# gorgonia/agogo

Hardware: AMD Instinct MI355X
Metric: mcts_sims_per_sec (higher is better)
Workload: dtype f32 (Winograd F(5x5,3x3): fp32 transforms; transform-domain products as fp16x2 = each fp32 operand scaled by a power of two and split into 2 fp16 pieces (22-23 significand bits, absolute error <= 2^-38 of the tensor range), 3 fp16 MFMAs per product, fp32 accumulate)

## Files before the change

agogo_amd/csrc/conv_wino_h2.hpp:

```cpp
#pragma once

template <int TM> struct WinoT;
template <> struct WinoT<4> {
  static constexpr int AL = 6, VSHIFT = 7;
  static constexpr float BT[6][6] = {{4, 0, -5, 0, 1, 0}, {0, -4, -4, 1, 1, 0}, {0, 4, -4, -1, 1, 0}, {0, -2, -1, 2, 1, 0}, {0, 2, -1, -2, 1, 0}, {0, 4, 0, -5, 0, 1}};
  static constexpr float AT[4][6] = {{1, 1, 1, 1, 1, 0}, {0, 1, -1, 2, -2, 0}, {0, 1, 1, 4, 4, 0}, {0, 1, -1, 8, -8, 1}};
  static constexpr double G[6][3] = {{1.0 / 4, 0, 0}, {-1.0 / 6, -1.0 / 6, -1.0 / 6}, {-1.0 / 6, 1.0 / 6, -1.0 / 6}, {1.0 / 24, 1.0 / 12, 1.0 / 6}, {1.0 / 24, -1.0 / 12, 1.0 / 6}, {0, 0, 1}};
};
template <> struct WinoT<5> {
  static constexpr int AL = 7, VSHIFT = 6;
  static constexpr float BT[7][7] = {{-0.5f, 0.25f, 2.5f, -1.25f, -2, 1, 0}, {0, 0.5f, 0.25f, -2.25f, -1, 1, 0}, {0, -0.5f, 0.75f, 1.75f, -3, 1, 0},
                                     {0, 1, 1.5f, -2, -1.5f, 1, 0},          {0, -1, 2.5f, 0, -2.5f, 1, 0},       {0, 0.25f, 0, -1.25f, 0, 1, 0},
                                     {0, -0.5f, 0.25f, 2.5f, -1.25f, -2, 1}};
  static constexpr float AT[5][7] = {{1, 1, 1, 1, 1, 1, 0}, {0, 1, -1, 0.5f, -0.5f, 2, 0}, {0, 1, 1, 0.25f, 0.25f, 4, 0}, {0, 1, -1, 0.125f, -0.125f, 8, 0},
                                     {0, 1, 1, 0.0625f, 0.0625f, 16, 1}};
  static constexpr double G[7][3] = {{-2, 0, 0}, {-2.0 / 3, -2.0 / 3, -2.0 / 3}, {-2.0 / 9, 2.0 / 9, -2.0 / 9}, {16.0 / 9, 8.0 / 9, 4.0 / 9}, {16.0 / 15, -8.0 / 15, 4.0 / 15},
                                     {2.0 / 45, 4.0 / 45, 8.0 / 45}, {0, 0, 1}};
};
template <int TM> __device__ __forceinline__ void wino_btv(const float* d, float* o);
template <int TM> __device__ __forceinline__ void wino_atv(const float* m, float* o);
template <> __device__ __forceinline__ void wino_btv<4>(const float* d, float* o) { wino_bt6(d, o); }
template <> __device__ __forceinline__ void wino_atv<4>(const float* m, float* o) { wino_at4(m, o); }
template <> __device__ __forceinline__ void wino_btv<5>(const float* d, float* o) {
  o[0] = -0.5f * d[0] + 0.25f * d[1] + 2.5f * d[2] - 1.25f * d[3] - 2.f * d[4] + d[5];
// ... 31 lines not shown
  const unsigned* amax_in;
  unsigned* amax_out;
  float* wave_max;
  float w_unscale;
  const float* t_in;
  const float* col_unscale;
  const float* t_next;
  int cform;
  const _Float16* U2c;
  const float* amax_true;
  const float* wm_prev;
  float* wm_out;
  unsigned* amax_next;
  float g1, g0;
  int gemm_variant;
  int temporal_stores;
  int live_r, live_c;
  int row_pad;
};
__device__ __forceinline__ size_t h2_row(const WinoH2Args& h, int pos, int t) {
  return (size_t)(t >> h.rsh) * h.rA + (size_t)pos * h.rB + (size_t)(t & h.rmask);
}

__device__ __forceinline__ void wino_h2_scales(unsigned amax_bits, int shift, float* s, float* inv) {
  int e = (int)((amax_bits >> 23) & 0xffu);
  if (amax_bits == 0u) { *s = 1.f; *inv = 1.f; return; }
  e = e < 30 ? 30 : (e > 230 ? 230 : e);
  *s = __uint_as_float((unsigned)(268 - shift - e) << 23);
  *inv = __uint_as_float((unsigned)(e - 14 + shift) << 23);
}
// ... 1072 lines not shown
```

agogo_amd/csrc/conv_wino_h2c.hpp:

```cpp
#pragma once

__device__ __forceinline__ unsigned h2c_img(int row, int slot) { return maps::h2c_img(row, slot); }

template <int NK, int PFA>
__global__ __launch_bounds__(256, 2) void wino_gemm_h2c_kernel(WinoH2Args h) {
  const WinoArgs& a = h.w;
  constexpr int SA = 128 * 128, SB = 256 * 128;
  __shared__ __attribute__((aligned(16))) unsigned char lds[SA + SB];

  const int n_nt = a.Ntot >> 8;
  const int per_pos = a.n_mtiles * n_nt;
  const int nblk = h.npos * per_pos;
  const int id = blockIdx.x;
  int q = nblk >> 3, rr = nblk & 7, xcd = id & 7, slot = id >> 3;
  int tile = (xcd < rr ? xcd * (q + 1) : rr * (q + 1) + (xcd - rr) * q) + slot;
  const int pos = tile / per_pos;
  const int rem = tile - pos * per_pos;
  const int m_tile = rem / n_nt, n_tile = rem - m_tile * n_nt;

  const int tid = threadIdx.x, lane = tid & 63, wid = tid >> 6;
  const int wm = wid >> 1, wn = wid & 1;
  const unsigned st_lds = h2c_img(tid >> 3, tid & 7);
  const char* abase = reinterpret_cast<const char*>(a.V) + ((size_t)m_tile * h.npos + pos) * (size_t)NK * SA + (size_t)tid * 16;
  const char* bbase = reinterpret_cast<const char*>(h.U2c) + (((size_t)pos * NK) * n_nt + n_tile) * (size_t)SB + (size_t)tid * 16;
// ... 521 lines not shown
template <> __device__ __forceinline__ void wino_atv_p<4>(const f2c* m, f2c* o) {
  const f2c s12 = m[1] + m[2], d12 = m[1] - m[2], s34 = m[3] + m[4], d34 = m[3] - m[4];
  o[0] = m[0] + s12 + s34;
  o[1] = d12 + 2.f * d34;
  o[2] = s12 + 4.f * s34;
  o[3] = d12 + 8.f * d34 + m[5];
}
template <> __device__ __forceinline__ void wino_atv_p<5>(const f2c* m, f2c* o) {
  const f2c s12 = m[1] + m[2], d12 = m[1] - m[2], s34 = m[3] + m[4], d34 = m[3] - m[4];
  o[0] = m[0] + s12 + s34 + m[5];
  o[1] = d12 + 0.5f * d34 + 2.f * m[5];
  o[2] = s12 + 0.25f * s34 + 4.f * m[5];
  o[3] = d12 + 0.125f * d34 + 8.f * m[5];
  o[4] = s12 + 0.0625f * s34 + 16.f * m[5] + m[6];
}
template <int TM> __device__ __forceinline__ void wino_at_acc_p(int nu, f2c* Y, f2c t);
template <> __device__ __forceinline__ void wino_at_acc_p<5>(int nu, f2c* Y, f2c t) {
  switch (nu) {
    case 0: Y[0] += t; break;
    case 1: Y[0] += t; Y[1] += t; Y[2] += t; Y[3] += t; Y[4] += t; break;
    case 2: Y[0] += t; Y[1] -= t; Y[2] += t; Y[3] -= t; Y[4] += t; break;
    case 3: Y[0] += t; Y[1] += 0.5f * t; Y[2] += 0.25f * t; Y[3] += 0.125f * t; Y[4] += 0.0625f * t; break;
    case 4: Y[0] += t; Y[1] -= 0.5f * t; Y[2] += 0.25f * t; Y[3] -= 0.125f * t; Y[4] += 0.0625f * t; break;
    case 5: Y[0] += t; Y[1] += 2.f * t; Y[2] += 4.f * t; Y[3] += 8.f * t; Y[4] += 16.f * t; break;
    default: Y[4] += t; break;
  }
}
template <> __device__ __forceinline__ void wino_at_acc_p<4>(int nu, f2c* Y, f2c t) {
  switch (nu) {
    case 0: Y[0] += t; break;
// ... 19 lines not shown
template <> __device__ __forceinline__ f2c wino_bt_row_p<4>(int i, const f2c* d) {
  switch (i) {
    case 0: return 4.f * d[0] - 5.f * d[2] + d[4];
    case 1: return -4.f * d[1] - 4.f * d[2] + d[3] + d[4];
    case 2: return 4.f * d[1] - 4.f * d[2] - d[3] + d[4];
    case 3: return -2.f * d[1] - d[2] + 2.f * d[3] + d[4];
    case 4: return 2.f * d[1] - d[2] - 2.f * d[3] + d[4];
    default: return 4.f * d[1] - 5.f * d[3] + d[5];
  }
}
template <int TM> __device__ __forceinline__ void wino_btv_p(const f2c* d, f2c* o) {
#pragma unroll
  for (int i = 0; i < TM + 2; i++) o[i] = wino_bt_row_p<TM>(i, d);
}

template <int TM, bool NT = true>
__global__ __launch_bounds__(256, 2) void wino_oip_h2c_kernel(WinoH2Args h) {
  constexpr int MAUX = 0, VAUX = NT ? 2 : 0;
  using WT = WinoT<TM>;
  constexpr int AL = WT::AL, NPRE = AL - 3;
  const WinoArgs& a = h.w;
  extern __shared__ __attribute__((aligned(16))) float ys[];
  const int tid = threadIdx.x, tl = tid >> 4, pr = tid & 15, lane = tid & 63;
  const int NS = a.C >> 5;
  const int PH = TM * a.nty + 2, PW = TM * a.ntx + 2;
  const int bpg = 16 / a.TPB;
  const int n_groups = (a.T + 15) >> 4, n_items = n_groups * NS;
  const int tt = tl % a.TPB, bl = tl / a.TPB;
  const int ty = tt / a.ntx, tx = tt - ty * a.ntx;
  for (int i = tid; i < bpg * PH * PW * 32; i += 256) ys[i] = 0.f;
  const __amdgpu_buffer_rsrc_t mr = h2_rsrc(a.Mb);
// ... 54 lines not shown
    for (int k = 0; k < TM; k++)
#pragma unroll
      for (int l = 0; l < TM; l++) { Y[k][l][0] = f2c{0.f, 0.f}; Y[k][l][1] = f2c{0.f, 0.f}; }
#pragma unroll
    for (int nu = 0; nu < AL; nu++) {
      f2c c0[AL], c1[AL], o0[TM], o1[TM];
#pragma unroll
      for (int xi = 0; xi < AL; xi++) {
        const float4 v = m[nu % NPRE][xi];
        c0[xi] = f2c{v.x, v.y}; c1[xi] = f2c{v.z, v.w};
      }
      if (nu + NPRE < AL) {
#pragma unroll
        for (int xi = 0; xi < AL; xi++) m[nu % NPRE][xi] = h2_ldf4<MAUX>(mr, m_voff(xi, nu + NPRE), m_soff(g, s, xi, nu + NPRE));
      }
      wino_atv_p<TM>(c0, o0);
      wino_atv_p<TM>(c1, o1);
#pragma unroll
      for (int k = 0; k < TM; k++) {
        f2c y0[TM], y1[TM];
#pragma unroll
        for (int l = 0; l < TM; l++) { y0[l] = Y[k][l][0]; y1[l] = Y[k][l][1]; }
        wino_at_acc_p<TM>(nu, y0, o0[k]);
        wino_at_acc_p<TM>(nu, y1, o1[k]);
#pragma unroll
        for (int l = 0; l < TM; l++) { Y[k][l][0] = y0[l]; Y[k][l][1] = y1[l]; }
      }
      __builtin_amdgcn_sched_barrier(0);
    }
    __builtin_amdgcn_sched_barrier(0);
    unsigned e_base = (unsigned)(32 * s + 2 * pr) * 16u + (unsigned)((TM * ty) * a.W + TM * tx) * e_pix;
    asm volatile("" : "+v"(e_base));
// ... 16 lines not shown
      if (k + 1 < TM) load_e((k + 1) & 1, k + 1);
#pragma unroll
      for (int l = 0; l < TM; l++) {
        const bool ok = live && ((okmask >> (k * TM + l)) & 1u);
        const float4 E0 = E[k & 1][l][0], E1 = E[k & 1][l][1];
        const f2c u0 = Y[k][l][0] * un0, u1 = Y[k][l][1] * un0;
        float va = u0.x * E0.x + E0.y, vb = u0.y * E0.z + E0.w;
        float vc = u1.x * E1.x + E1.y, vd = u1.y * E1.z + E1.w;
        va = va > 0.f ? va : 0.f; vb = vb > 0.f ? vb : 0.f; vc = vc > 0.f ? vc : 0.f; vd = vd > 0.f ? vd : 0.f;
        const float y0 = ok ? va + vb : 0.f, y1 = ok ? vc + vd : 0.f;
        *reinterpret_cast<float2*>(yw + ((k + 1) * PW + l + 1) * 32) = make_float2(y0, y1);
        mxv = fmaxf(mxv, fmaxf(y0, y1));
      }
      __builtin_amdgcn_sched_barrier(0);
    }
#pragma unroll
    for (int o = 8; o > 0; o >>= 1) mxv = fmaxf(mxv, __shfl_xor(mxv, o, 64));
    if (pr == 0 && live) h.wm_out[(size_t)t * NS + s] = mxv;
    float ax;
    if (h.amax_true) ax = __uint_as_float(reinterpret_cast<const unsigned*>(h.amax_true)[b]);
    else {
      const int wmpb = a.TPB * NS;
      const float* wp = h.wm_prev + (size_t)b * wmpb;
      ax = 0.f;
      for (int i = pr; i < wmpb; i += 16) ax = fmaxf(ax, wp[i]);
#pragma unroll
      for (int o = 8; o > 0; o >>= 1) ax = fmaxf(ax, __shfl_xor(ax, o, 64));
    }
    const float bound = h.g1 * ax + h.g0;
    const unsigned bbits = __float_as_uint(bound);
    if (s == 0 && tt == 0 && pr == 0 && live) h.amax_next[b] = bbits;
    float sb, inv_;
    wino_h2_scales(bbits, WT::VSHIFT, &sb, &inv_);
    const float sv = live ? sb : 0.f;
    __syncthreads();
    {
      const int nx = item + (int)gridDim.x < n_items ? item + (int)gridDim.x : item;
      const int g2 = __builtin_amdgcn_readfirstlane(nx / NS), s2 = __builtin_amdgcn_readfirstlane(nx - (nx / NS) * NS);
#pragma unroll
      for (int nu = 0; nu < NPRE; nu++)
#pragma unroll
        for (int xi = 0; xi < AL; xi++) m[nu][xi] = h2_ldf4<MAUX>(mr, m_voff(xi, nu), m_soff(g2, s2, xi, nu));
    }
    __builtin_amdgcn_sched_barrier(0);
    const unsigned v_base = (unsigned)((((g >> 3) * h.npos) * NS + s)) * 16384u;
    const unsigned v_g = (unsigned)(g & 7) * 2048u, v_g_r = (unsigned)(g & 7) * (gr_r * 128u), v_g_c = (unsigned)(g & 7) * (gr_c * 128u);
    const unsigned v_pos = (unsigned)NS * 16384u;
    const float* yr = ybase;
    asm volatile("" : "+v"(yr));
#pragma unroll
    for (int i0 = 0; i0 < AL; i0 += 3) {
      constexpr int NRMAX = 3;
      const int nr = AL - i0 < NRMAX ? AL - i0 : NRMAX;
      f2c tmr[NRMAX][AL];
#pragma unroll
      for (int j = 0; j < AL; j++) {
        f2c d[AL];
#pragma unroll
        for (int ii = 0; ii < AL; ii++) {
// ... 59 lines not shown
  h.tm = tm; h.npos = (tm + 2) * (tm + 2);
  a.nty = ceil_div(a.H, tm); a.ntx = ceil_div(a.W, tm); a.TPB = a.nty * a.ntx; a.T = a.B * a.TPB;
  h.rsh = 7; h.rmask = 127; h.rA = (unsigned)h.npos * 128u; h.rB = 128u;
  a.n_mtiles = ceil_div(a.T, 128); a.n_ntiles = ceil_div(a.Ntot, 128);
  h.in_swap = 1; h.cform = 1; h.wm_per_board = 0;
}
constexpr int WINO_H2_GEMM_DEFAULT = 1;
static inline int wino_h2c_gemm_variant(const WinoH2Args& h) { return h.gemm_variant > 0 ? h.gemm_variant : WINO_H2_GEMM_DEFAULT; }
static inline bool wino_h2c_dma_ok(const WinoH2Args& h) {
  return wino_h2_rows(h.npos, (size_t)h.w.T) * h.w.C * 4 < ((size_t)1 << 31) && (size_t)h.npos * h.w.C * h.w.Ntot * 4 < ((size_t)1 << 31);
}
static inline bool wino_h2c_fits31(const WinoH2Args& h) { return wino_h2_rows(h.npos, (size_t)h.w.T) * h.w.Ntot * 4 < ((size_t)1 << 31); }
static bool wino_h2c_oip_ready(agz_ctx* ctx) {
  if (!(ctx->func_attr_state & 2u)) {
    const bool ok = hipFuncSetAttribute(reinterpret_cast<const void*>(&wino_oip_h2c_kernel<5>), hipFuncAttributeMaxDynamicSharedMemorySize, 80 * 1024) == hipSuccess &&
                    hipFuncSetAttribute(reinterpret_cast<const void*>(&wino_oip_h2c_kernel<4>), hipFuncAttributeMaxDynamicSharedMemorySize, 80 * 1024) == hipSuccess;
    if (!ok) (void)hipGetLastError();
    ctx->func_attr_state |= 2u | (ok ? 1u : 0u);
  }
  return (ctx->func_attr_state & 1u) != 0;
}
static void wino_h2c_rows(agz_ctx* ctx, WinoH2Args& h, int oi_variant, bool keep_all) {
  wino_h2c_geometry(h);
  h.live_r = h.live_c = 0;
  const int gemm = wino_h2c_gemm_variant(h) & 15;
  const maps::WinoRows g = maps::wino_rows(h.w.H, h.w.W, h.tm);
  if (keep_all || gemm != 1 || oi_variant != 4 || !wino_h2c_dma_ok(h) || !wino_h2c_fits31(h) || !maps::rows_short_ok(g) || !wino_h2c_oip_ready(ctx)) return;
  h.live_r = g.dead_y ? maps::rows_slot_live(g, maps::ROWS_R) : 0;
  h.live_c = g.dead_x ? maps::rows_slot_live(g, maps::ROWS_C) : 0;
}
static void wino_h2c_in(agz_ctx* ctx, WinoH2Args& h, hipStream_t st) {
// ... 33 lines not shown
  }
  switch (h.w.C >> 5) {
    case 4: hipLaunchKernelGGL((wino_gemm_h2c_kernel<4, 2>), g, dim3(256), 0, st, h); break;
    case 8: hipLaunchKernelGGL((wino_gemm_h2c_kernel<8, 2>), g, dim3(256), 0, st, h); break;
    case 12: hipLaunchKernelGGL((wino_gemm_h2c_kernel<12, 2>), g, dim3(256), 0, st, h); break;
    default: hipLaunchKernelGGL((wino_gemm_h2c_kernel<16, 2>), g, dim3(256), 0, st, h); break;
  }
}
static void wino_h2c_oi(agz_ctx* ctx, WinoH2Args& h, bool last, hipStream_t st, int variant = 4) {
  wino_h2c_geometry(h);
  ProfScopeOn ps(ctx, AGZ_PROF_WINO_OUT, st == ctx->stream.raw());
  const WinoArgs& a = h.w;
  const dim3 g((unsigned)ceil_div(a.T, 16), (unsigned)(a.C >> 5));
  const size_t shm = last ? 0 : (size_t)(16 / a.TPB) * a.H * a.W * 32 * sizeof(float);
  const bool fits31 = wino_h2c_fits31(h);
  if (variant == 4 && !last && fits31 && wino_h2c_oip_ready(ctx)) {
    const size_t shp = (size_t)(16 / a.TPB) * (h.tm * a.nty + 2) * (h.tm * a.ntx + 2) * 32 * sizeof(float);
    const int items = ceil_div(a.T, 16) * (a.C >> 5);
    const dim3 gp((unsigned)std::min(items, 2 * ctx->num_cus));
    if (h.tm == 5 && h.temporal_stores) {
      (void)hipFuncSetAttribute(reinterpret_cast<const void*>(&wino_oip_h2c_kernel<5, false>), hipFuncAttributeMaxDynamicSharedMemorySize, 80 * 1024);
      hipLaunchKernelGGL((wino_oip_h2c_kernel<5, false>), gp, dim3(256), shp, st, h);
      return;
    }
    if (h.tm == 5) hipLaunchKernelGGL((wino_oip_h2c_kernel<5>), gp, dim3(256), shp, st, h);
    else hipLaunchKernelGGL((wino_oip_h2c_kernel<4>), gp, dim3(256), shp, st, h);
    return;
  }
  if (h.tm == 5) {
    if (last) hipLaunchKernelGGL((wino_oi_h2c_kernel<5, true>), g, dim3(256), shm, st, h);
    else hipLaunchKernelGGL((wino_oi_h2c_kernel<5, false>), g, dim3(256), shm, st, h);
  } else {
    if (last) hipLaunchKernelGGL((wino_oi_h2c_kernel<4, true>), g, dim3(256), shm, st, h);
    else hipLaunchKernelGGL((wino_oi_h2c_kernel<4, false>), g, dim3(256), shm, st, h);
// ... 3 lines not shown
```

agogo_amd/csrc/conv_x3.hpp:

```cpp
#pragma once

typedef short bf16x8_t __attribute__((ext_vector_type(8)));
typedef unsigned u32x4_t __attribute__((ext_vector_type(4)));

__device__ __forceinline__ void x3_split(float v, unsigned& h, unsigned& m, unsigned& l) {
  unsigned hu = __float_as_uint(v) & 0xffff0000u;
  float r = v - __uint_as_float(hu);
  unsigned mu = __float_as_uint(r) & 0xffff0000u;
  float r2 = r - __uint_as_float(mu);
  h = hu; m = mu; l = __float_as_uint(r2);
}
__device__ __forceinline__ unsigned x3_pack(unsigned e0, unsigned e1) { return __builtin_amdgcn_perm(e1, e0, 0x07060302u); }

__device__ __forceinline__ unsigned x3_lds_off(int row, int half) { return (unsigned)(row * 32 + ((half ^ ((row >> 3) & 1)) << 4)); }

__device__ __forceinline__ void x3_amax_flush(unsigned* amax, int b, float m, int lane) {
#pragma unroll
  for (int o = 16; o > 0; o >>= 1) m = fmaxf(m, __shfl_xor(m, o, 64));
  if ((lane & 31) == 0) atomicMax(&amax[b], __float_as_uint(m));
}
#define X3_EPILOGUE \
  int amx_b = -1; float amx_m = 0.f;    \
  _Pragma("unroll") \
  for (int i = 0; i < 2; i++) { \
// ... 30 lines not shown
              a.y[obase + c] = acc[i][j][r]; \
            } else { \
              float2 e = reinterpret_cast<const float2*>(a.ep)[(size_t)p * a.Cout_p + c]; \
              float v = acc[i][j][r] * e.x + e.y; \
              v = v > 0.f ? v : 0.f; \
              a.y[obase + c] = v; \
              amx_m = fmaxf(amx_m, v); \
            } \
          } \
        } \
      } \
    } \
  } \
  if (!DUAL && a.amax_out && amx_b >= 0) x3_amax_flush(a.amax_out, amx_b, amx_m, lane);

template <bool DUAL>
__global__ __launch_bounds__(256, 3) void conv3x3_x3_kernel(ConvArgs a, const unsigned short* __restrict__ w3) {
  constexpr int BM = 128, BNT = 128;
  constexpr int PIECE = 128 * 32;
  constexpr int STAGE = 6 * PIECE;
  __shared__ __attribute__((aligned(16))) unsigned char lds[2 * STAGE];

  const int nblk = a.n_mtiles * a.n_ntiles;
  const int id = blockIdx.x;
  int q = nblk >> 3, rr = nblk & 7, xcd = id & 7, slot = id >> 3;
  int tile = (xcd < rr ? xcd * (q + 1) : rr * (q + 1) + (xcd - rr) * q) + slot;
  const int m_tile = tile / a.n_ntiles, n_tile = tile - m_tile * a.n_ntiles;
  const int m0 = m_tile * BM, n0 = n_tile * BNT;

  const int tid = threadIdx.x, lane = tid & 63, wid = tid >> 6;
// ... 100 lines not shown
    X3_STORE_B(XB0, XB1, XB2, (BUF) ^ 1) X3_SB                                               \
    X3_QUAD(0, 1) X3_QUAD(0, 0) X3_SB                                                        \
    __syncthreads();                                                                         \
  }

  X3_GLOAD(ya0, ya1, yb0, yb1, yb2)
  X3_GLOAD(xa0, xa1, xb0, xb1, xb2)
  X3_STORE_A(ya0, ya1, 0)
  X3_STORE_B(yb0, yb1, yb2, 0)
  __syncthreads();
  for (int it = 0; it < NK; it += 2) {
    X3_ITER(0, xa0, xa1, xb0, xb1, xb2, ya0, ya1, yb0, yb1, yb2)
    if (it + 1 < NK) X3_ITER(1, ya0, ya1, yb0, yb1, yb2, xa0, xa1, xb0, xb1, xb2)
  }

  X3_EPILOGUE
}
```

agogo_amd/csrc/net.hip:

```cpp
#include "net.hpp"
#include "gemm_maps.hpp"

#include <cmath>
#include <cstdio>
#include <cstring>
#include <type_traits>

typedef float f32x16 __attribute__((ext_vector_type(16)));
typedef float f32x4 __attribute__((ext_vector_type(4)));

namespace agz {

struct ConvArgs {
  const float* x;
  const float* w;
  const void* ep;
  float* y;
  int M, HW, W, Wp, HpWp;
  int Cin_p, Cout_p, Ntot;
  int n_mtiles, n_ntiles;
  int raw;
  int splits;
  int per;
  float* ws;
  const unsigned* amax_in;
  float w_unscale;
  const unsigned* w_amax_dev;
  unsigned* amax_out;
};

__device__ __forceinline__ int swz_off(int row, int chunk) { return row * 32 + ((chunk ^ ((row >> 1) & 7)) << 2); }

template <int WM, int WN, int MT, bool DUAL>
__device__ __forceinline__ void conv_tile(const ConvArgs& a, float* lds, const int m0, const int n_tile, const int split) {
  constexpr int BM = WM * MT * 32;
  constexpr int BNT = WN * 64;
  static_assert(WM * WN == 4, "4 waves");
  constexpr int STAGE = (BM + BNT) * 32;
  const int n0 = n_tile * BNT;

  const int tid = threadIdx.x, lane = tid & 63, wid = tid >> 6;
  const int wm = wid / WN, wn = wid % WN;

// ... 1046 lines not shown
    wino_v_cap = t.v_elems * t.n_scr; wino_chunk_cap = 0;
  }
  const size_t need_amax = (size_t)(conf.SharedLayers + 1) * B + t.wm_board * B;
  if (need_amax > amax_cap) {
    AGZ_HIP_TRY(hipStreamSynchronize(ctx->stream));
    if (ctx->stream2) AGZ_HIP_TRY(hipStreamSynchronize(ctx->stream2));
    if (d_amax) hipFree(d_amax);
    d_amax = nullptr; amax_cap = 0;
    AGZ_HIP_TRY(hipMalloc(&d_amax, need_amax * sizeof(unsigned)));
    amax_cap = need_amax;
    if (amax_moved) *amax_moved = true;
  }
  return AGZ_OK;
}

void agz_net::wino_h2c_block(int l, int B, int b0, int ci, const H2Tower& t, hipStream_t st, float* cur, float* nxt) {
  const size_t wmb = (size_t)t.tpb * (Kp >> 5);
  const bool last = l + 1 == conf.SharedLayers;
  float* d_wave_max = reinterpret_cast<float*>(d_amax + (size_t)(conf.SharedLayers + 1) * B);
  WinoH2Args hh{};
  WinoArgs& wa = hh.w;
  wa.x = cur + (size_t)b0 * Hp * Wp * Kp; wa.y = nxt + (size_t)b0 * Hp * Wp * Kp;
  wa.V = d_wV + (size_t)ci * t.v_elems; wa.Mb = d_wM + (size_t)ci * t.m_elems; wa.ep = d_ep_h2[l];
  wa.B = std::min(t.chunk, B - b0); wa.H = H; wa.W = W; wa.Hp = Hp; wa.Wp = Wp; wa.C = Kp; wa.Cout_p = Kp; wa.Ntot = 2 * Kp;
  hh.U2c = d_u2c_dual[l]; hh.w_unscale = 1.f; hh.tm = wino_tm;
  hh.amax_in = d_amax + (size_t)l * B + b0;
  hh.amax_next = last ? nullptr : d_amax + (size_t)(l + 1) * B + b0;
  hh.amax_true = l == 0 ? reinterpret_cast<const float*>(d_amax + b0) : nullptr;
  hh.wm_prev = d_wave_max + ((size_t)((l + 1) & 1) * B + b0) * wmb;
  hh.wm_out = d_wave_max + ((size_t)(l & 1) * B + b0) * wmb;
  hh.g1 = wino_g1[l]; hh.g0 = wino_g0[l];
  {
    static const int gemm_env = [] {
      const char* e = getenv("AGZ_WINO_H2_GEMM");
      const int v = e ? atoi(e) : 0;
      if (v == 0 || (((v & 63) == 1 || (v & 63) == 2) && (v >> 6) <= 3)) return v;
      fprintf(stderr, "libagz: AGZ_WINO_H2_GEMM=%s ignored (want 1 or 2, optionally + 64 and / or + 128)\n", e);
      return 0;
    }();
    const int gv = wino_gemm > 0 ? wino_gemm : gemm_env;
    hh.gemm_variant = gv & 63; hh.temporal_stores = (gv >> 6) & 1;
    agz::wino_h2c_rows(ctx, hh, t.form_want == 1 ? 1 : 4, ((gv >> 7) & 1) != 0);
    wino_live_r = hh.live_r; wino_live_c = hh.live_c;
  }
  if (l == 0) agz::wino_h2c_in(ctx, hh, st);
  agz::wino_h2c_gemm(ctx, hh, st);
  agz::wino_h2c_oi(ctx, hh, last, st, t.form_want == 1 ? 1 : 4);
}

void agz_net::heads_spread_range(agz::HeadArgs h, bool nb4, int B, int b0, int nb, hipStream_t st) {
  h.x += (size_t)b0 * Hp * Wp * Kp;
  h.feat = d_hs + (size_t)b0 * 3 * HW; h.cols = d_hs + (size_t)B * 3 * HW + (size_t)b0 * (conf.ActionSpace + conf.FC);
  h.policy += (size_t)b0 * conf.ActionSpace; h.value += b0;
  hipLaunchKernelGGL(heads_feat_kernel, dim3(ceil_div(HW, 4), nb), dim3(256), 0, st, h);
  if (nb4)
    hipLaunchKernelGGL(heads_fc_nb_kernel<4>, dim3(ceil_div(conf.ActionSpace + conf.FC, 64), ceil_div(nb, 4)), dim3(1024), 0, st, h, nb);
  else
    hipLaunchKernelGGL(heads_fc_kernel, dim3(ceil_div(conf.ActionSpace + conf.FC, 64), nb), dim3(1024), 0, st, h);
  hipLaunchKernelGGL(heads_out_kernel, dim3(nb), dim3(256), 0, st, h);
}

// ... 24 lines not shown
  }
  return AGZ_OK;
}

int agz_net::forward_half(int B, int half, hipStream_t st, float* policy_dev, float* value_dev, hipEvent_t mid) {
  const int nb = B / 2, b0 = half * nb;
  const FwdPlan plan = fwd_plan(B);
  const H2Tower t = wino_h2_tower(B);
  ConvArgs a{};
  a.M = nb * HW; a.HW = HW; a.W = W; a.Wp = Wp; a.HpWp = Hp * Wp;
  a.x = d_act_in + (size_t)b0 * Hp * Wp * Fp; a.w = d_w_init; a.ep = d_ep_init_h2; a.y = d_actA + (size_t)b0 * Hp * Wp * Kp;
  a.Cin_p = Fp; a.Cout_p = Kp; a.Ntot = Kp;
  a.n_ntiles = ceil_div(a.Ntot, 128); a.n_mtiles = ceil_div(a.M, 128);
  a.splits = 1; a.per = 0; a.ws = nullptr; a.raw = 0;
  AGZ_HIP_TRY(hipMemsetAsync(d_amax + b0, 0, (size_t)nb * sizeof(unsigned), st));
  a.amax_out = d_amax + b0;
  hipLaunchKernelGGL((conv3x3_x3_kernel<false>), dim3(a.n_mtiles * a.n_ntiles), dim3(256), 0, st, a, d_w3_init);
  const int L = conf.SharedLayers;
  for (int l = 0; l < L; l++) {
    wino_h2c_block(l, B, b0, half, t, st, d_actA, d_actB);
    if (mid && l == L / 2) AGZ_HIP_TRY(hipEventRecord(mid, st));
  }
  HeadArgs h{};
  h.x = d_actB; h.conv = d_head_conv; h.bn = d_head_bn; h.Wp = d_Wp; h.bp = d_bp; h.W1 = d_W1; h.b1 = d_b1; h.W2 = d_W2;
  h.b2 = d_b2; h.policy = policy_dev; h.value = value_dev;
  h.H = H; h.W = W; h.HW = HW; h.Wp_ = Wp; h.HpWp = Hp * Wp; h.Kp = Kp; h.A = conf.ActionSpace; h.FC = conf.FC;
  heads_spread_range(h, plan.heads_nb, B, b0, nb, st);
  AGZ_HIP_TRY(hipGetLastError());
  return AGZ_OK;
}

// ... 33 lines not shown
    lat_wmax_cap = B;
  }
  int rc;
  bool amax0_done = false;
  if (lat_in) {
    agz::LatInArgs li{};
    li.x = d_act_in; li.w = d_w_init_t; li.ep = reinterpret_cast<const float2*>(d_ep_init); li.t = d_lat_tin[0]; li.y = d_actA; li.words = d_lat_wmax[1];
    li.B = B; li.H = H; li.W = W; li.Hp = Hp; li.Wp = Wp; li.Cout_p = Kp; li.groups_per_board = in_groups;
    ProfScope ps(ctx, AGZ_PROF_CONV_INIT);
    hipLaunchKernelGGL(agz::lat_input_kernel, dim3(Kp / 64, B * in_groups), dim3(256), 0, ctx->stream, li);
    rc = AGZ_OK;
  }
  else if (split_ok && compute_mode != AGZ_COMPUTE_F32_MFMA && d_w3_init && Kp % 128 == 0 &&
      (size_t)B * Hp * Wp * Fp * sizeof(float) < ((size_t)1 << 32)) {
    a.n_ntiles = ceil_div(a.Ntot, 128); a.n_mtiles = ceil_div(a.M, 128);
    a.splits = 1; a.per = 0; a.ws = nullptr; a.raw = 0;
    ProfScope ps(ctx, AGZ_PROF_CONV_INIT);
    if (wino_h2_ok && d_amax && amax_cap >= (size_t)B) {
      AGZ_HIP_TRY(hipMemsetAsync(d_amax, 0, (size_t)B * sizeof(unsigned), ctx->stream));
      a.amax_out = d_amax; amax0_done = true;
    }
    hipLaunchKernelGGL((conv3x3_x3_kernel<false>), dim3(a.n_mtiles * a.n_ntiles), dim3(256), 0, ctx->stream, a, d_w3_init);
    a.amax_out = nullptr;
    rc = AGZ_OK;
  }
  else if (cfg != 0) rc = launch_conv<4, 1, 1, false>(ctx, a, wsp, &ws_cap);
  else if (half_init) rc = launch_conv<2, 2, 1, false>(ctx, a, wsp, &ws_cap);
  else rc = launch_conv<2, 2, 2, false>(ctx, a, wsp, &ws_cap);
  if (rc != AGZ_OK) return rc;
  float* cur = d_actA;
  float* nxt = d_actB;
// ... 514 lines not shown
int agz_net_min_same_batch(agz_net* n, int k, int G, int* batch) {
  AGZ_REQUIRE(n && batch && k >= 1 && G >= k, AGZ_E_INVALID, "agz_net_min_same_batch: bad argument");
  AGZ_REQUIRE(n->committed, AGZ_E_STATE, "agz_net_min_same_batch: commit the net first");
  *batch = n->min_same_batch(k, G);
  return AGZ_OK;
}

int agz_net_wino_h2_last_rows(agz_net* n, int* live_r, int* live_c) {
  AGZ_REQUIRE(n && live_r && live_c, AGZ_E_INVALID, "agz_net_wino_h2_last_rows: null argument");
  *live_r = n->wino_live_r; *live_c = n->wino_live_c;
  return AGZ_OK;
}

int agz_net_set_wino_h2_gemm(agz_net* n, int variant) {
  AGZ_REQUIRE(n, AGZ_E_INVALID, "agz_net_set_wino_h2_gemm: null net");
  AGZ_REQUIRE(((variant & 63) <= 2 && (variant >> 6) <= 3) || ((variant & 15) == 2 && (variant >> 4) <= 3), AGZ_E_INVALID, "agz_net_set_wino_h2_gemm: variant %d (want 0, 1, 2, + 64, + 128, or 2 + 16 * mode)", variant);
  n->wino_gemm = variant;
  return AGZ_OK;
}

int agz_wino_stages(agz_ctx* ctx, const float* x, const float* w, int B, int H, int W, int C, int N, float* V, float* M) {
  AGZ_REQUIRE(ctx && x && w && V && M, AGZ_E_INVALID, "agz_wino_stages: NULL argument");
  AGZ_REQUIRE(B >= 1 && H >= 1 && W >= 1 && C >= 16 && C % 16 == 0 && N >= 1, AGZ_E_INVALID, "agz_wino_stages: bad shape");
  AGZ_HIP_TRY(hipSetDevice(ctx->device));
  const int Hp = H + 2, Wp = W + 2;
  std::vector<float> xp((size_t)B * Hp * Wp * C, 0.f);
  for (int b = 0; b < B; b++) for (int h = 0; h < H; h++)
    memcpy(&xp[(((size_t)b * Hp + h + 1) * Wp + 1) * C], &x[((size_t)b * H + h) * W * C], (size_t)W * C * sizeof(float));
  std::vector<unsigned short> u3;
  agz::wino_build_u3(u3, N, C, [&](int n, int ci, int tap) -> double { return (double)w[((size_t)n * C + ci) * 9 + tap]; });
  agz::WinoArgs a{};
// ... 128 lines not shown
```

agogo_amd/csrc/net.hpp:

```cpp
#pragma once
#include <string>
#include <vector>

#include "common.hpp"

namespace agz {
struct Param {
  std::string name;
  std::vector<float> v;
  std::vector<int> ref_shape;
  int kind;
};
struct BNStats { std::vector<float> mean, var; };
int conv3x3_raw(agz_ctx* ctx, const float* x, const float* w, float* y, int B, int H, int W, int Cin_p, int Cout_p);
int conv3x3_raw_x3(agz_ctx* ctx, const float* x, const unsigned short* w3, float* y, int B, int H, int W, int Cin_p, int Cout_p);
int split_w3(agz_ctx* ctx, const float* w, unsigned short* w3, int N, int Cin_p);
inline size_t w3_elems(int N, int Cin_p) { return (size_t)9 * 3 * N * Cin_p; }
struct WinoRawScratch {
  float* V = nullptr; float* M = nullptr; void* U2 = nullptr; unsigned* words = nullptr;
  size_t v_cap = 0, m_cap = 0, u_cap = 0; int b_cap = 0;
  void* w2 = nullptr; unsigned* h2_words = nullptr;
  size_t w2_cap = 0; int h2_b_cap = 0, h2_flip = 0;
};
int conv3x3_raw_h2(agz_ctx* ctx, const float* x, const float* w, float* y, int B, int H, int W, int Cin_p, int Cout_p, WinoRawScratch* sc,
// ... 28 lines not shown
  float* d_ep_init = nullptr;
  unsigned short* d_w3_init = nullptr;
  std::vector<float*> d_w_dual;
  std::vector<float*> d_ep_dual;
  std::vector<unsigned short*> d_w3_dual;
  std::vector<_Float16*> d_w2_dual;
  std::vector<float> w_unscale;
  std::vector<unsigned short*> d_u3_dual;
  std::vector<_Float16*> d_u2_dual;
  std::vector<float> u_unscale;
  std::vector<float*> d_u2_tin;
  std::vector<float*> d_u2_colun;
  std::vector<_Float16*> d_u2c_dual;
  std::vector<float> wino_g1, wino_g0;
  int wino_gemm = 0;
  int wino_live_r = 0, wino_live_c = 0;
  int wino_form = -1;
  void free_u2c() { for (auto& p : d_u2c_dual) if (p) hipFree(p); d_u2c_dual.clear(); wino_g1.clear(); wino_g0.clear(); }
  int build_wino_h2_weights();
  int wino_tm = 4;
  size_t wino_v_cap = 0;
  float* d_wV = nullptr;
  float* d_wM = nullptr;
  int wino_chunk_cap = 0;
  int build_wino_weights();
  unsigned* d_amax = nullptr;
  size_t amax_cap = 0;
  int compute_mode = AGZ_COMPUTE_F32_MFMA;
  bool compute_force = false;
  float* d_head_conv = nullptr;
// ... 47 lines not shown
```

Before: 44300.

## Route last Winograd layer through OIP kernel and add row-wise x3 epilogue

Adds a LAST template variant of the in-place output-transform kernel that skips the amax/scale computation for the next layer and writes the final tower output directly from shared memory. It also adds a row-wise epilogue for the initial x3 conv that uses permlane32 swaps and readlane-indexed per-row epilogue params, plus a new gemm-word bit (256) that selects the old paths. By default (bit clear) the last layer now uses the OIP path and the x3 kernel uses the new epilogue. The aim is to avoid a separate slower last-layer output kernel and unnecessary amax work, at the cost of extra kernel instantiations and a scalar-heavy epilogue.

Result: no change. 44470 (median of 6 runs) (+0.4%).

```diff
diff --git a/agogo_amd/csrc/conv_wino_h2.hpp b/agogo_amd/csrc/conv_wino_h2.hpp
--- a/agogo_amd/csrc/conv_wino_h2.hpp
+++ b/agogo_amd/csrc/conv_wino_h2.hpp
@@ -69,6 +69,7 @@
   unsigned* amax_next;
   float g1, g0;
   int gemm_variant;
+  int last_plain;
   int temporal_stores;
   int live_r, live_c;
   int row_pad;
diff --git a/agogo_amd/csrc/conv_wino_h2c.hpp b/agogo_amd/csrc/conv_wino_h2c.hpp
--- a/agogo_amd/csrc/conv_wino_h2c.hpp
+++ b/agogo_amd/csrc/conv_wino_h2c.hpp
@@ -559,6 +559,12 @@
   o[3] = d12 + 0.125f * d34 + 8.f * m[5];
   o[4] = s12 + 0.0625f * s34 + 16.f * m[5] + m[6];
 }
+__device__ __forceinline__ void wino_atv_p4_seq(const f2c* m, f2c* o) {
+  o[0] = m[0] + m[1] + m[2] + m[3] + m[4];
+  o[1] = m[1] - m[2] + 2.f * m[3] - 2.f * m[4];
+  o[2] = m[1] + m[2] + 4.f * m[3] + 4.f * m[4];
+  o[3] = m[1] - m[2] + 8.f * m[3] - 8.f * m[4] + m[5];
+}
 template <int TM> __device__ __forceinline__ void wino_at_acc_p(int nu, f2c* Y, f2c t);
 template <> __device__ __forceinline__ void wino_at_acc_p<5>(int nu, f2c* Y, f2c t) {
   switch (nu) {
@@ -608,7 +614,7 @@
   for (int i = 0; i < TM + 2; i++) o[i] = wino_bt_row_p<TM>(i, d);
 }
 
-template <int TM, bool NT = true>
+template <int TM, bool NT = true, bool LAST = false>
 __global__ __launch_bounds__(256, 2) void wino_oip_h2c_kernel(WinoH2Args h) {
   constexpr int MAUX = 0, VAUX = NT ? 2 : 0;
   using WT = WinoT<TM>;
@@ -693,8 +699,8 @@
 #pragma unroll
         for (int xi = 0; xi < AL; xi++) m[nu % NPRE][xi] = h2_ldf4<MAUX>(mr, m_voff(xi, nu + NPRE), m_soff(g, s, xi, nu + NPRE));
       }
-      wino_atv_p<TM>(c0, o0);
-      wino_atv_p<TM>(c1, o1);
+      if constexpr (LAST && TM == 4) { wino_atv_p4_seq(c0, o0); wino_atv_p4_seq(c1, o1); }
+      else { wino_atv_p<TM>(c0, o0); wino_atv_p<TM>(c1, o1); }
 #pragma unroll
       for (int k = 0; k < TM; k++) {
         f2c y0[TM], y1[TM];
@@ -741,25 +747,28 @@
       }
       __builtin_amdgcn_sched_barrier(0);
     }
-#pragma unroll
-    for (int o = 8; o > 0; o >>= 1) mxv = fmaxf(mxv, __shfl_xor(mxv, o, 64));
-    if (pr == 0 && live) h.wm_out[(size_t)t * NS + s] = mxv;
-    float ax;
-    if (h.amax_true) ax = __uint_as_float(reinterpret_cast<const unsigned*>(h.amax_true)[b]);
-    else {
-      const int wmpb = a.TPB * NS;
-      const float* wp = h.wm_prev + (size_t)b * wmpb;
-      ax = 0.f;
-      for (int i = pr; i < wmpb; i += 16) ax = fmaxf(ax, wp[i]);
-#pragma unroll
-      for (int o = 8; o > 0; o >>= 1) ax = fmaxf(ax, __shfl_xor(ax, o, 64));
-    }
-    const float bound = h.g1 * ax + h.g0;
-    const unsigned bbits = __float_as_uint(bound);
-    if (s == 0 && tt == 0 && pr == 0 && live) h.amax_next[b] = bbits;
-    float sb, inv_;
-    wino_h2_scales(bbits, WT::VSHIFT, &sb, &inv_);
-    const float sv = live ? sb : 0.f;
+    float sv = 0.f;
+    if constexpr (!LAST) {
+#pragma unroll
+      for (int o = 8; o > 0; o >>= 1) mxv = fmaxf(mxv, __shfl_xor(mxv, o, 64));
+      if (pr == 0 && live) h.wm_out[(size_t)t * NS + s] = mxv;
+      float ax;
+      if (h.amax_true) ax = __uint_as_float(reinterpret_cast<const unsigned*>(h.amax_true)[b]);
+      else {
+        const int wmpb = a.TPB * NS;
+        const float* wp = h.wm_prev + (size_t)b * wmpb;
+        ax = 0.f;
+        for (int i = pr; i < wmpb; i += 16) ax = fmaxf(ax, wp[i]);
+#pragma unroll
+        for (int o = 8; o > 0; o >>= 1) ax = fmaxf(ax, __shfl_xor(ax, o, 64));
+      }
+      const float bound = h.g1 * ax + h.g0;
+      const unsigned bbits = __float_as_uint(bound);
+      if (s == 0 && tt == 0 && pr == 0 && live) h.amax_next[b] = bbits;
+      float sb, inv_;
+      wino_h2_scales(bbits, WT::VSHIFT, &sb, &inv_);
+      sv = live ? sb : 0.f;
+    }
     __syncthreads();
     {
       const int nx = item + (int)gridDim.x < n_items ? item + (int)gridDim.x : item;
@@ -770,6 +779,20 @@
         for (int xi = 0; xi < AL; xi++) m[nu][xi] = h2_ldf4<MAUX>(mr, m_voff(xi, nu), m_soff(g2, s2, xi, nu));
     }
     __builtin_amdgcn_sched_barrier(0);
+    if constexpr (LAST) {
+      const int HW = a.H * a.W, npix = bpg * HW, sub = tid & 7;
+      for (int idx = tid >> 3; idx < npix; idx += 32) {
+        const int lb = idx / HW, p = idx - lb * HW;
+        const int hh = p / a.W, ww = p - hh * a.W;
+        const int bb = g * bpg + lb;
+        if (bb < a.B) {
+          const float4 v = *reinterpret_cast<const float4*>(ys + ((size_t)(lb * PH + hh + 1) * PW + ww + 1) * 32 + sub * 4);
+          *reinterpret_cast<float4*>(a.y + ((size_t)bb * a.Hp * a.Wp + (size_t)(hh + 1) * a.Wp + (ww + 1)) * a.Cout_p + 32 * s + sub * 4) = v;
+        }
+      }
+      __syncthreads();
+      continue;
+    }
     const unsigned v_base = (unsigned)((((g >> 3) * h.npos) * NS + s)) * 16384u;
     const unsigned v_g = (unsigned)(g & 7) * 2048u, v_g_r = (unsigned)(g & 7) * (gr_r * 128u), v_g_c = (unsigned)(g & 7) * (gr_c * 128u);
     const unsigned v_pos = (unsigned)NS * 16384u;
@@ -859,7 +882,9 @@
 static bool wino_h2c_oip_ready(agz_ctx* ctx) {
   if (!(ctx->func_attr_state & 2u)) {
     const bool ok = hipFuncSetAttribute(reinterpret_cast<const void*>(&wino_oip_h2c_kernel<5>), hipFuncAttributeMaxDynamicSharedMemorySize, 80 * 1024) == hipSuccess &&
-                    hipFuncSetAttribute(reinterpret_cast<const void*>(&wino_oip_h2c_kernel<4>), hipFuncAttributeMaxDynamicSharedMemorySize, 80 * 1024) == hipSuccess;
+                    hipFuncSetAttribute(reinterpret_cast<const void*>(&wino_oip_h2c_kernel<4>), hipFuncAttributeMaxDynamicSharedMemorySize, 80 * 1024) == hipSuccess &&
+                    hipFuncSetAttribute(reinterpret_cast<const void*>(&wino_oip_h2c_kernel<5, true, true>), hipFuncAttributeMaxDynamicSharedMemorySize, 80 * 1024) == hipSuccess &&
+                    hipFuncSetAttribute(reinterpret_cast<const void*>(&wino_oip_h2c_kernel<4, true, true>), hipFuncAttributeMaxDynamicSharedMemorySize, 80 * 1024) == hipSuccess;
     if (!ok) (void)hipGetLastError();
     ctx->func_attr_state |= 2u | (ok ? 1u : 0u);
   }
@@ -923,10 +948,15 @@
   const dim3 g((unsigned)ceil_div(a.T, 16), (unsigned)(a.C >> 5));
   const size_t shm = last ? 0 : (size_t)(16 / a.TPB) * a.H * a.W * 32 * sizeof(float);
   const bool fits31 = wino_h2c_fits31(h);
-  if (variant == 4 && !last && fits31 && wino_h2c_oip_ready(ctx)) {
+  if (variant == 4 && !(last && h.last_plain) && fits31 && wino_h2c_oip_ready(ctx)) {
     const size_t shp = (size_t)(16 / a.TPB) * (h.tm * a.nty + 2) * (h.tm * a.ntx + 2) * 32 * sizeof(float);
     const int items = ceil_div(a.T, 16) * (a.C >> 5);
     const dim3 gp((unsigned)std::min(items, 2 * ctx->num_cus));
+    if (last) {
+      if (h.tm == 5) hipLaunchKernelGGL((wino_oip_h2c_kernel<5, true, true>), gp, dim3(256), shp, st, h);
+      else hipLaunchKernelGGL((wino_oip_h2c_kernel<4, true, true>), gp, dim3(256), shp, st, h);
+      return;
+    }
     if (h.tm == 5 && h.temporal_stores) {
       (void)hipFuncSetAttribute(reinterpret_cast<const void*>(&wino_oip_h2c_kernel<5, false>), hipFuncAttributeMaxDynamicSharedMemorySize, 80 * 1024);
       hipLaunchKernelGGL((wino_oip_h2c_kernel<5, false>), gp, dim3(256), shp, st, h);
diff --git a/agogo_amd/csrc/conv_x3.hpp b/agogo_amd/csrc/conv_x3.hpp
--- a/agogo_amd/csrc/conv_x3.hpp
+++ b/agogo_amd/csrc/conv_x3.hpp
@@ -68,6 +68,54 @@
   } \
   if (!DUAL && a.amax_out && amx_b >= 0) x3_amax_flush(a.amax_out, amx_b, amx_m, lane);
 
+template <bool MULTI>
+__device__ __forceinline__ void x3_rows_epilogue(const ConvArgs& a, f32x16 (&acc)[2][2], const int c, const int lane, const int r_b,
+                                                 const int r_p, const int r_pix, const unsigned long long valid) {
+  const bool cok = c < a.Cout_p;
+  const unsigned cl = (unsigned)(cok ? c : a.Cout_p - 1);
+  const float2* ep = reinterpret_cast<const float2*>(a.ep);
+  int amx_b = MULTI ? -1 : __builtin_amdgcn_readlane(r_b, 0);
+  float amx_m = 0.f;
+  float2 E[2][8];
+  auto load_e = [&](int buf, int g) {
+#pragma unroll
+    for (int u = 0; u < 8; u++) E[buf][u] = (ep + (size_t)__builtin_amdgcn_readlane(r_p, g * 8 + u) * a.Cout_p)[cl];
+  };
+  load_e(0, 0);
+#pragma unroll
+  for (int g = 0; g < 8; g++) {
+    if (g + 1 < 8) load_e((g + 1) & 1, g + 1);
+#pragma unroll
+    for (int u = 0; u < 4; u++) {
+      const int i = g >> 2, r = 4 * (g & 3) + u;
+      const auto s32 = __builtin_amdgcn_permlane32_swap(__float_as_uint(acc[i][0][r]), __float_as_uint(acc[i][1][r]), false, false);
+      acc[i][0][r] = __uint_as_float(s32[0]);
+      acc[i][1][r] = __uint_as_float(s32[1]);
+    }
+#pragma unroll
+    for (int u = 0; u < 8; u++) {
+      const int k = g * 8 + u, q = k & 31;
+      const float x = acc[k >> 5][(q >> 2) & 1][(q & 3) + 4 * (q >> 3)];
+      const bool live = (valid >> k) & 1ull;
+      if (MULTI) {
+        const int b = __builtin_amdgcn_readlane(r_b, k);
+        if (a.amax_out && live && b != amx_b) {
+          if (amx_b >= 0) x3_amax_flush(a.amax_out, amx_b, amx_m, lane);
+          amx_b = b; amx_m = 0.f;
+        }
+      }
+      const float2 e = E[g & 1][u];
+      float v = x * e.x + e.y;
+      v = v > 0.f ? v : 0.f;
+      if (live && cok) {
+        (a.y + (size_t)__builtin_amdgcn_readlane(r_pix, k) * a.Cout_p)[cl] = v;
+        amx_m = fmaxf(amx_m, v);
+      }
+    }
+  }
+  if (a.amax_out && (MULTI ? amx_b >= 0 : valid != 0ull)) x3_amax_flush(a.amax_out, amx_b, amx_m, lane);
+}
+
 template <bool DUAL>
 __global__ __launch_bounds__(256, 3) void conv3x3_x3_kernel(ConvArgs a, const unsigned short* __restrict__ w3) {
   constexpr int BM = 128, BNT = 128;
@@ -198,5 +246,21 @@
     if (it + 1 < NK) X3_ITER(1, ya0, ya1, yb0, yb1, yb2, xa0, xa1, xb0, xb1, xb2)
   }
 
+  if constexpr (!DUAL) {
+    if (!a.raw && !a.ep_per_element) {
+      const int wv = __builtin_amdgcn_readfirstlane(wm);
+      int m = m0 + wv * 64 + lane;
+      const bool mvalid = m < a.M;
+      if (!mvalid) m = a.M - 1;
+      const int b = m / a.HW, p = m - b * a.HW;
+      const int h = p / a.W, w = p - h * a.W;
+      const int pix = b * a.HpWp + (h + 1) * a.Wp + (w + 1);
+      const unsigned long long valid = __ballot(mvalid);
+      const int c = n0 + wn * 64 + lane;
+      if (__builtin_amdgcn_readlane(b, 0) != __builtin_amdgcn_readlane(b, 63)) x3_rows_epilogue<true>(a, acc, c, lane, b, p, pix, valid);
+      else x3_rows_epilogue<false>(a, acc, c, lane, b, p, pix, valid);
+      return;
+    }
+  }
   X3_EPILOGUE
 }
diff --git a/agogo_amd/csrc/net.hip b/agogo_amd/csrc/net.hip
--- a/agogo_amd/csrc/net.hip
+++ b/agogo_amd/csrc/net.hip
@@ -27,6 +27,7 @@
   float w_unscale;
   const unsigned* w_amax_dev;
   unsigned* amax_out;
+  int ep_per_element;
 };
 
 __device__ __forceinline__ int swz_off(int row, int chunk) { return row * 32 + ((chunk ^ ((row >> 1) & 7)) << 2); }
@@ -1103,6 +1104,17 @@
   return AGZ_OK;
 }
 
+int agz_net::wino_gemm_word() const {
+  static const int gemm_env = [] {
+    const char* e = getenv("AGZ_WINO_H2_GEMM");
+    const int v = e ? atoi(e) : 0;
+    if (v == 0 || (v > 0 && (v & 63) <= 2 && (v >> 6) <= 7)) return v;
+    fprintf(stderr, "libagz: AGZ_WINO_H2_GEMM=%s ignored (want 0, 1 or 2, optionally + 64, + 128 and / or + 256)\n", e);
+    return 0;
+  }();
+  return wino_gemm > 0 ? wino_gemm : gemm_env;
+}
+
 void agz_net::wino_h2c_block(int l, int B, int b0, int ci, const H2Tower& t, hipStream_t st, float* cur, float* nxt) {
   const size_t wmb = (size_t)t.tpb * (Kp >> 5);
   const bool last = l + 1 == conf.SharedLayers;
@@ -1120,20 +1132,14 @@
   hh.wm_out = d_wave_max + ((size_t)(l & 1) * B + b0) * wmb;
   hh.g1 = wino_g1[l]; hh.g0 = wino_g0[l];
   {
-    static const int gemm_env = [] {
-      const char* e = getenv("AGZ_WINO_H2_GEMM");
-      const int v = e ? atoi(e) : 0;
-      if (v == 0 || (((v & 63) == 1 || (v & 63) == 2) && (v >> 6) <= 3)) return v;
-      fprintf(stderr, "libagz: AGZ_WINO_H2_GEMM=%s ignored (want 1 or 2, optionally + 64 and / or + 128)\n", e);
-      return 0;
-    }();
-    const int gv = wino_gemm > 0 ? wino_gemm : gemm_env;
+    const int gv = wino_gemm_word();
     hh.gemm_variant = gv & 63; hh.temporal_stores = (gv >> 6) & 1;
     agz::wino_h2c_rows(ctx, hh, t.form_want == 1 ? 1 : 4, ((gv >> 7) & 1) != 0);
     wino_live_r = hh.live_r; wino_live_c = hh.live_c;
   }
   if (l == 0) agz::wino_h2c_in(ctx, hh, st);
   agz::wino_h2c_gemm(ctx, hh, st);
+  hh.last_plain = ends_before();
   agz::wino_h2c_oi(ctx, hh, last, st, t.form_want == 1 ? 1 : 4);
 }
 
@@ -1188,7 +1194,7 @@
   a.n_ntiles = ceil_div(a.Ntot, 128); a.n_mtiles = ceil_div(a.M, 128);
   a.splits = 1; a.per = 0; a.ws = nullptr; a.raw = 0;
   AGZ_HIP_TRY(hipMemsetAsync(d_amax + b0, 0, (size_t)nb * sizeof(unsigned), st));
-  a.amax_out = d_amax + b0;
+  a.amax_out = d_amax + b0; a.ep_per_element = ends_before();
   hipLaunchKernelGGL((conv3x3_x3_kernel<false>), dim3(a.n_mtiles * a.n_ntiles), dim3(256), 0, st, a, d_w3_init);
   const int L = conf.SharedLayers;
   for (int l = 0; l < L; l++) {
@@ -1252,7 +1258,7 @@
   else if (split_ok && compute_mode != AGZ_COMPUTE_F32_MFMA && d_w3_init && Kp % 128 == 0 &&
       (size_t)B * Hp * Wp * Fp * sizeof(float) < ((size_t)1 << 32)) {
     a.n_ntiles = ceil_div(a.Ntot, 128); a.n_mtiles = ceil_div(a.M, 128);
-    a.splits = 1; a.per = 0; a.ws = nullptr; a.raw = 0;
+    a.splits = 1; a.per = 0; a.ws = nullptr; a.raw = 0; a.ep_per_element = ends_before();
     ProfScope ps(ctx, AGZ_PROF_CONV_INIT);
     if (wino_h2_ok && d_amax && amax_cap >= (size_t)B) {
       AGZ_HIP_TRY(hipMemsetAsync(d_amax, 0, (size_t)B * sizeof(unsigned), ctx->stream));
@@ -1797,7 +1803,7 @@
 
 int agz_net_set_wino_h2_gemm(agz_net* n, int variant) {
   AGZ_REQUIRE(n, AGZ_E_INVALID, "agz_net_set_wino_h2_gemm: null net");
-  AGZ_REQUIRE(((variant & 63) <= 2 && (variant >> 6) <= 3) || ((variant & 15) == 2 && (variant >> 4) <= 3), AGZ_E_INVALID, "agz_net_set_wino_h2_gemm: variant %d (want 0, 1, 2, + 64, + 128, or 2 + 16 * mode)", variant);
+  AGZ_REQUIRE(variant >= 0 && (((variant & 63) <= 2 && (variant >> 6) <= 7) || ((variant & 15) == 2 && (variant >> 4) <= 3)), AGZ_E_INVALID, "agz_net_set_wino_h2_gemm: variant %d (want 0, 1, 2, + 64, + 128, + 256, or 2 + 16 * mode)", variant);
   n->wino_gemm = variant;
   return AGZ_OK;
 }
diff --git a/agogo_amd/csrc/net.hpp b/agogo_amd/csrc/net.hpp
--- a/agogo_amd/csrc/net.hpp
+++ b/agogo_amd/csrc/net.hpp
@@ -66,6 +66,8 @@
   std::vector<_Float16*> d_u2c_dual;
   std::vector<float> wino_g1, wino_g0;
   int wino_gemm = 0;
+  int wino_gemm_word() const;
+  bool ends_before() const { return ((wino_gemm_word() >> 8) & 1) != 0; }
   int wino_live_r = 0, wino_live_c = 0;
   int wino_form = -1;
   void free_u2c() { for (auto& p : d_u2c_dual) if (p) hipFree(p); d_u2c_dual.clear(); wino_g1.clear(); wino_g0.clear(); }
```
